# liangxuy/ReGenNet

Hardware: AMD Instinct MI355X
Metric: sampled motions/sec (higher is better)
Workload: dtype bf16 MFMA operands, fp32 accumulate/LayerNorm/softmax, for 990 of 1000 steps; fp16 MFMA operands for the next 8; split-bf16 (x3) for the last 2; 1 GPU; ntu: [B=256/GPU,56,6,60] online/concat/no_cond L8 d512, 1000-step DDPM, Philox noise, hipGraph=on; batch_per_gpu=256, global_batch=256, denoiser_evals_per_motion=1000, parallelism=batch-shard x1

## Files before the change

### regennet_amd/csrc/rgn_device.h

```cpp
#pragma once
#include <hip/hip_runtime.h>

#include <type_traits>
#include <utility>

#include "rgn_internal.h"
#include "rgn_layout.h"

#define RGN_AS1 __attribute__((address_space(1)))
#define RGN_AS3 __attribute__((address_space(3)))

namespace rgn {
namespace {

template <class T, int N>
using vec_t = T __attribute__((ext_vector_type(N)));
typedef vec_t<float, 2> f32x2;
typedef vec_t<float, 4> f32x4;
typedef vec_t<float, 16> f32x16;
typedef vec_t<__bf16, 2> bf16x2;
typedef vec_t<__bf16, 4> bf16x4;
typedef vec_t<__bf16, 8> bf16x8;
typedef vec_t<_Float16, 2> f16x2;
typedef vec_t<_Float16, 8> f16x8;
typedef vec_t<unsigned int, 2> u32x2;
typedef vec_t<unsigned int, 4> u32x4;

template <int N>
__device__ __forceinline__ void wait_vmcnt() {
    asm volatile("s_waitcnt vmcnt(%0)" ::"n"(N > 63 ? 63 : N) : "memory");
}
template <int N>
__device__ __forceinline__ void wait_lgkmcnt() {
    static_assert(N >= 0 && N <= 15, "lgkmcnt is a four-bit counter");
    asm volatile("s_waitcnt lgkmcnt(%0)" ::"n"(N) : "memory");
}

template <int CTRL>
__device__ __forceinline__ float dpp(float v) {
    return __builtin_bit_cast(float, __builtin_amdgcn_update_dpp(0, __builtin_bit_cast(int, v), CTRL, 0xf, 0xf, true));
}
__device__ __forceinline__ float row16_sum(float v) {
    v += dpp<0xB1>(v);
    v += dpp<0x4E>(v);
    v += dpp<0x141>(v);
    v += dpp<0x140>(v);
    return v;
}
__device__ __forceinline__ float wave_sum_dpp(float v) {
    const int b = __builtin_bit_cast(int, row16_sum(v));
    return __builtin_bit_cast(float, __builtin_amdgcn_readlane(b, 0)) + __builtin_bit_cast(float, __builtin_amdgcn_readlane(b, 16)) +
           __builtin_bit_cast(float, __builtin_amdgcn_readlane(b, 32)) + __builtin_bit_cast(float, __builtin_amdgcn_readlane(b, 48));
}
__device__ __forceinline__ float wave_sum_shfl(float v) {
#pragma unroll
    for (int o = 32; o > 0; o >>= 1) v += __shfl_xor(v, o, 64);
    return v;
}
__device__ __forceinline__ float wave_max_shfl(float v) {
#pragma unroll
    for (int o = 32; o > 0; o >>= 1) v = fmaxf(v, __shfl_xor(v, o, 64));
    return v;
}

template <int... Is, class F>
__device__ __forceinline__ void static_for_seq(std::integer_sequence<int, Is...>, F&& f) { (f(std::integral_constant<int, Is>{}), ...); }
template <int N, class F>
__device__ __forceinline__ void static_for(F&& f) { static_for_seq(std::make_integer_sequence<int, N>{}, static_cast<F&&>(f)); }

__device__ __forceinline__ void split_bf16(const f32x4 v, bf16x4& hi, bf16x4& lo) {
#pragma unroll
    for (int j = 0; j < 4; ++j) {
        const __bf16 h = (__bf16)v[j];
        hi[j] = h;
        lo[j] = (__bf16)(v[j] - (float)h);
    }
}
__device__ __forceinline__ void split_bf16(const float (&v)[8], bf16x8& hi, bf16x8& lo) {
#pragma unroll
    for (int j = 0; j < 8; ++j) {
        hi[j] = (__bf16)v[j];
        lo[j] = (__bf16)(v[j] - (float)hi[j]);
    }
}
__device__ __forceinline__ void plane_put(const Planes& p, int row, int col, float v) {
    const size_t o = plane_off(p.rows, row, col);
    const __bf16 h = (__bf16)v;
    p.hi[o] = h;
    if (p.lo) p.lo[o] = (__bf16)(v - (float)h);
}

__device__ __forceinline__ float erf_as(float x) {
    const float ax = fabsf(x);
    const float t = __frcp_rn(fmaf(0.3275911f, ax, 1.0f));
    float p = fmaf(1.061405429f, t, -1.453152027f);
    p = fmaf(p, t, 1.421413741f);
    p = fmaf(p, t, -0.284496736f);
    p = fmaf(p, t, 0.254829592f);
    const float e = 1.0f - p * t * __expf(-ax * ax);
    return copysignf(e, x);
}
__device__ __forceinline__ float erf_as_rcpf(float x) {
    const float ax = fabsf(x);
    const float t = __builtin_amdgcn_rcpf(fmaf(0.3275911f, ax, 1.0f));
    float p = fmaf(1.061405429f, t, -1.453152027f);
    p = fmaf(p, t, 1.421413741f);
    p = fmaf(p, t, -0.284496736f);
    p = fmaf(p, t, 0.254829592f);
    const float e = 1.0f - p * t * __expf(-ax * ax);
    return copysignf(e, x);
}
__device__ __forceinline__ float gelu_as(float v) { return v * 0.5f * (1.0f + erf_as(v * 0.70710678118654752440f)); }
__device__ __forceinline__ float gelu_as_rcpf(float v) { return v * 0.5f * (1.0f + erf_as_rcpf(v * 0.70710678118654752440f)); }

__device__ __forceinline__ f32x2 gelu2_p13(f32x2 x) {
    const f32x2 t = {__builtin_amdgcn_fmed3f(x[0], -3.9f, 3.9f), __builtin_amdgcn_fmed3f(x[1], -3.9f, 3.9f)};
    const f32x2 z = t * t;
    f32x2 p = f32x2{3.214928057e-08f, 3.214928057e-08f};
    p = __builtin_elementwise_fma(p, z, f32x2{-2.075321845e-06f, -2.075321845e-06f});
    p = __builtin_elementwise_fma(p, z, f32x2{5.740237248e-05f, 5.740237248e-05f});
    p = __builtin_elementwise_fma(p, z, f32x2{-9.056383278e-04f, -9.056383278e-04f});
    p = __builtin_elementwise_fma(p, z, f32x2{9.218782187e-03f, 9.218782187e-03f});
    p = __builtin_elementwise_fma(p, z, f32x2{-6.556465477e-02f, -6.556465477e-02f});
    p = __builtin_elementwise_fma(p, z, f32x2{3.986084461e-01f, 3.986084461e-01f});
    return x * __builtin_elementwise_fma(t, p, f32x2{0.5f, 0.5f});
}
__device__ __forceinline__ f32x2 gelu2_p15(f32x2 x) {
    f32x2 u = x * 0.70710678118654752440f;
    u = __builtin_elementwise_min(__builtin_elementwise_max(u, f32x2{-3.2f, -3.2f}), f32x2{3.2f, 3.2f});
    const f32x2 z = u * u;
    f32x2 p = f32x2{-2.6911866e-07f, -2.6911866e-07f};
    p = __builtin_elementwise_fma(p, z, f32x2{1.2661994e-05f, 1.2661994e-05f});
    p = __builtin_elementwise_fma(p, z, f32x2{-2.5566161e-04f, -2.5566161e-04f});
    p = __builtin_elementwise_fma(p, z, f32x2{2.9286479e-03f, 2.9286479e-03f});
    p = __builtin_elementwise_fma(p, z, f32x2{-2.1317327e-02f, -2.1317327e-02f});
    p = __builtin_elementwise_fma(p, z, f32x2{1.0528564e-01f, 1.0528564e-01f});
    p = __builtin_elementwise_fma(p, z, f32x2{-3.7135834e-01f, -3.7135834e-01f});
    p = __builtin_elementwise_fma(p, z, f32x2{1.1274883e+00f, 1.1274883e+00f});
    const f32x2 hx = x * 0.5f;
    return __builtin_elementwise_fma(hx, p * u, hx);
}

template <bool F16> struct OpFmt;
template <> struct OpFmt<false> {
    typedef __bf16 t;
    typedef __bf16 v8 __attribute__((ext_vector_type(8)));
    typedef __bf16 v4 __attribute__((ext_vector_type(4)));
    typedef float acc16 __attribute__((ext_vector_type(16)));
    static __device__ __forceinline__ acc16 mfma(v8 a, v8 b, acc16 c) { return __builtin_amdgcn_mfma_f32_32x32x16_bf16(a, b, c, 0, 0, 0); }
};
template <> struct OpFmt<true> {
    typedef _Float16 t;
    typedef _Float16 v8 __attribute__((ext_vector_type(8)));
    typedef _Float16 v4 __attribute__((ext_vector_type(4)));
    typedef float acc16 __attribute__((ext_vector_type(16)));
    static __device__ __forceinline__ acc16 mfma(v8 a, v8 b, acc16 c) { return __builtin_amdgcn_mfma_f32_32x32x16_f16(a, b, c, 0, 0, 0); }
};

__device__ __forceinline__ int xcd_affine(int bid, int nwg) {
    const int q8 = nwg >> 3, r8 = nwg & 7, xcd = bid & 7;
    return (xcd < r8 ? xcd * (q8 + 1) : r8 * (q8 + 1) + (xcd - r8) * q8) + (bid >> 3);
}

__device__ __forceinline__ void half_swap(float& a, float& b) { asm volatile("s_nop 1\n\tv_permlane32_swap_b32 %0, %1\n\ts_nop 1" : "+v"(a), "+v"(b)); }
__device__ __forceinline__ float half_max(float v) {
    float o = v;
    asm volatile("" : "+v"(o));
    half_swap(v, o);
    return fmaxf(v, o);
}
__device__ __forceinline__ float half_sum(float v) {
    float o = v;
    asm volatile("" : "+v"(o));
    half_swap(v, o);
    return v + o;
}

template <int AUX = 0, int NKB = 16, int NW = 8, class T>
__device__ __forceinline__ void tile_dma_in(char* img, const T* plane, int rows, size_t row0, int live, int lane, int wave) {
    const int r16 = lane >> 2, c = lane & 3;
#pragma unroll
    for (int j = 0; j < 4 * NKB / NW; ++j) {
        const int p = wave + NW * j, kb = p >> 2, r = (p & 3) * 16 + r16;
        const int rr = r < live ? r : live - 1;
        const size_t src = plane_chunk(rows, row0 + rr, kb, img_dma_chunk(r, c));
        __builtin_amdgcn_global_load_lds((const RGN_AS1 void*)(plane + src), (RGN_AS3 void*)(img + p * 1024), 16, 0, AUX);
    }
}

__device__ __forceinline__ void rot6d_to_matrix(float a1x, float a1y, float a1z, float a2x, float a2y, float a2z, float* m) {
    float n1 = fmaxf(sqrtf(a1x * a1x + a1y * a1y + a1z * a1z), 1e-12f);
    const float b1x = a1x / n1, b1y = a1y / n1, b1z = a1z / n1;
    const float dot = b1x * a2x + b1y * a2y + b1z * a2z;
    float b2x = a2x - dot * b1x, b2y = a2y - dot * b1y, b2z = a2z - dot * b1z;
    const float n2 = fmaxf(sqrtf(b2x * b2x + b2y * b2y + b2z * b2z), 1e-12f);
    b2x /= n2; b2y /= n2; b2z /= n2;
    m[0] = b1x; m[1] = b1y; m[2] = b1z;
    m[3] = b2x; m[4] = b2y; m[5] = b2z;
    m[6] = b1y * b2z - b1z * b2y;
    m[7] = b1z * b2x - b1x * b2z;
    m[8] = b1x * b2y - b1y * b2x;
}

template <class F>
auto dispatch_bools(F&& f) { return f(); }
template <class F, class... Rest>
auto dispatch_bools(F&& f, bool b, Rest... rest) {
    auto bind = [&](auto B) { return dispatch_bools([&](auto... bs) { return f(B, bs...); }, rest...); };
    return b ? bind(std::true_type{}) : bind(std::false_type{});
}

}
}
```

### regennet_amd/csrc/rgn_layers.hip

```cpp
#include "rgn_internal.h"
#include "rgn_device.h"
#include "rgn_tail.h"
#include "rgn_sampler.h"

#include <hip/hip_runtime.h>

#include <cmath>
#include <type_traits>
#include <utility>

namespace rgn {

#ifndef RGN_LY_ST_AUX
#define RGN_LY_ST_AUX 16
#endif

constexpr int LY_NTH = 512, LY_KB = 4096;
constexpr int LY_X = 0, LY_Y = 64 * 1024, LY_EXCH = LY_Y, LY_RED = 128 * 1024, LY_REDF = 2 * 8 * 64, LY_VEC = LY_RED + 2 * LY_REDF * 4, LY_VECW = 640,
              LY_LDS = 160 * 1024;
constexpr int LY_PF = LY_VEC + 8 * LY_VECW * 4;
static_assert(LY_PF + 8 * 256 <= LY_LDS, "LDS map");
enum { V_BO = 0, V_G1 = 64, V_G2 = 128, V_B2 = 192, V_SPV = 256, V_BF1 = 320 , V_BF2 = 448, V_G3 = 512, V_B3 = 576 };
constexpr int LY_RDA = 6;
constexpr int LY_RDM = 8;
struct LYT {
    static constexpr int MT = 2, NT = 2, NW = 8, R = 64, RD = LY_RDM, KB = LY_KB, RED = LY_RED, REDF = LY_REDF;
};

#ifdef RGN_LY_STAMPS
__device__ long long g_ly_st[1024][16];
#define RGN_LYT(i)                                                                                   \
    {                                                                                                \
        __builtin_amdgcn_sched_barrier(0);                                                           \
        if (threadIdx.x == 0 && blockIdx.x < 1024 && l == RGN_LY_STAMPS) g_ly_st[blockIdx.x][i] = __builtin_readcyclecounter(); \
        __builtin_amdgcn_sched_barrier(0);                                                           \
    }
#define RGN_LYS(i)                                                                                   \
    {                                                                                                \
        __builtin_amdgcn_sched_barrier(0);                                                           \
        if (threadIdx.x == 0 && blockIdx.x < 1024 && it == 1) g_ly_st[blockIdx.x][i] = __builtin_readcyclecounter(); \
        __builtin_amdgcn_sched_barrier(0);                                                           \
    }
#else
#define RGN_LYT(i)
#define RGN_LYS(i)
#endif

constexpr int LY_XLD = 356, LY_TILE = 0, LY_XIMG = 92160, LY_NKX = 11;
static_assert(64 * LY_XLD * 4 <= LY_XIMG && LY_XIMG + LY_NKX * 4096 <= LY_LDS, "step boundary LDS map");

template <bool STEPS, bool GUIDED = false, bool F16 = false, bool INPAINT = false>
__global__ __launch_bounds__(LY_NTH, 2) void k_layers(LayersArgs g) {
    static_assert(STEPS || !GUIDED, "guidance inside the launch needs the step boundary");
    static_assert(STEPS || !INPAINT, "in-painting (rgn_set_inpainting) belongs to the step boundary");
    using OP = OpFmt<F16>;
    using op_t = typename OP::t;
    using op8 = typename OP::v8;
    using op4 = typename OP::v4;
    extern __shared__ __attribute__((aligned(16))) char smem[];
    const int tid = threadIdx.x, lane = tid & 63;
    const int wave = __builtin_amdgcn_readfirstlane(tid >> 6);
    const int wn = wave & 3, hg = wave >> 2;
    const int l31 = lane & 31, kh = lane >> 5;
    const int b = xcd_affine(blockIdx.x, gridDim.x), Tq = g.Tq;
    const size_t row0 = (size_t)b * Tq;
#ifdef RGN_LY_PRIO
    if (wave >= 4) __builtin_amdgcn_s_setprio(RGN_LY_PRIO);
#endif
    float* vec = reinterpret_cast<float*>(smem + LY_VEC) + wave * LY_VECW;
    const int lane16 = lane * 16;
    tile_dma_in(smem + LY_X, g.h, g.rows, row0, Tq, lane, wave);
    const int first_step = (g.stepvec || STEPS) ? *g.d_step : 0;
    const TailLane tl = tail_lane<LYT>(smem, lane, wave);
    static_assert(LY_X == 0, "a_off addresses the image at byte 0");
    int a_off[2], a_offy[2];
    tail_a_off(a_off, lane);
    tail_a_off(a_offy, a_off, LY_Y);
    using Pass = TailPass;
    op8 wf[LY_RDM][2];
    const float qs2 = g.qscale * 1.44269504088896340736f;

    f32x4 qb[4];
    float vb1;
    auto load_qbias = [&](const float* bqkv, int r) {
        const float* bq = bqkv + (2 * r + hg) * 128 + wn * 32;
#pragma unroll
        for (int i4 = 0; i4 < 4; ++i4) qb[i4] = *reinterpret_cast<const f32x4*>(bq + 8 * i4 + 4 * kh);
        vb1 = bq[1024 + l31];
    };

    wait_vmcnt<0>();
    __builtin_amdgcn_s_barrier();
    load_qbias(g.lw[0].bqkv, 0);

    const int nit = STEPS ? g.steps : 1;
    auto out_proj = [&](f32x16 (&acc)[2][2], int wv) {
#pragma unroll
        for (int a2 = 0; a2 < 2; ++a2)
#pragma unroll
            for (int b2 = 0; b2 < 2; ++b2)
#pragma unroll
                for (int i = 0; i < 16; ++i) acc[a2][b2][i] = 0.f;
        if (wv < 6) {
            const int cb0 = 2 * wv;
            const Pass p_out{__builtin_amdgcn_make_buffer_rsrc(const_cast<__bf16*>(g.Wout) + (size_t)cb0 * 1024, 0, (16 * g.nb_out - cb0) * 2048, 0x00020000), LY_NKX * 2048, 0};
#pragma unroll
            for (int s2 = 0; s2 < LY_RDM - 1; ++s2) tail_load_g<OP, LYT>(wf, tl, p_out, s2, s2);
            tail_gemm<OP, LYT, 32, false, 0>(acc, wf, tl, a_off, p_out, p_out);
        }
    };
    for (int it = 0; it < nit; ++it) {
    const int step = first_step - it;
    for (int pass = 0; pass < (GUIDED ? 2 : 1); ++pass) {
    if (GUIDED && pass == 1) {
        f32x16 accp[2][2];
        int wave_p = wave, lane_p = lane, b_p = b;
        asm volatile("" : "+s"(wave_p), "+s"(b_p));
        asm volatile("" : "+v"(lane_p));
        out_proj(accp, wave_p);
        if (wave_p < 6) {
            float* pk = g.park + ((size_t)b_p * 6 + wave_p) * 4096 + lane_p * 4;
#pragma unroll
            for (int nt = 0; nt < 2; ++nt)
#pragma unroll
                for (int mt = 0; mt < 2; ++mt)
#pragma unroll
                    for (int i4 = 0; i4 < 4; ++i4)
                        *reinterpret_cast<f32x4*>(pk + ((nt * 2 + mt) * 4 + i4) * 256) = f32x4{accp[nt][mt][4 * i4], accp[nt][mt][4 * i4 + 1], accp[nt][mt][4 * i4 + 2], accp[nt][mt][4 * i4 + 3]};
        }
        __builtin_amdgcn_s_barrier();
        tile_dma_in<16>(smem + LY_X, g.h, g.rows, g.half + (size_t)b_p * Tq, Tq, lane_p, wave_p);
        wait_vmcnt<0>();
        __builtin_amdgcn_s_barrier();
    }
    for (int l = 0; l < g.L; ++l) {
        const LayerWts& w = g.lw[l];
        RGN_LYT(0)
        op4 attk[2][2][4];
        float bo_r = 0.f;
        {
            struct PassA { __amdgpu_buffer_rsrc_t rs; };
            auto qrs = [&](int r) {
                const int blk = (2 * r + hg) * 4 + wn;
                return __builtin_amdgcn_make_buffer_rsrc(const_cast<__bf16*>(w.Wqkv) + (size_t)blk * 1024, 0, 3 * 512 * 512 * 2 - blk * 2048, 0x00020000);
            };
            const PassA pa[2] = {{qrs(0)}, {qrs(1)}};
            op8 wq[LY_RDA][3];
            auto load_ga = [&](const PassA& ps, int hs, int slot) {
                int soff;
                asm volatile("s_mov_b32 %0, %1" : "=s"(soff) : "i"(frag_granule(hs, 48 * 2048)));
#pragma unroll
                for (int t = 0; t < 3; ++t)
                    wq[slot][t] = __builtin_bit_cast(op8, __builtin_amdgcn_raw_buffer_load_b128(ps.rs, lane16, soff + t * (16 * 2048), 0));
            };
            constexpr int AH = LY_RDA - 1;
#pragma unroll
            for (int s = 0; s < AH; ++s) load_ga(pa[0], s, s);
#pragma unroll
            for (int r = 0; r < 2; ++r) {
                const int head = 2 * r + hg;
                f32x16 acc[2][3];
#pragma unroll
                for (int ta = 0; ta < 2; ++ta)
#pragma unroll
                    for (int i4 = 0; i4 < 4; ++i4)
#pragma unroll
                        for (int e = 0; e < 4; ++e) {
                            acc[ta][0][4 * i4 + e] = qb[i4][e];
                            acc[ta][1][4 * i4 + e] = 0.f;
                            acc[ta][2][4 * i4 + e] = vb1;
                        }
                __builtin_amdgcn_sched_barrier(0);
                {
                    op8 af[2];
#pragma unroll
                    for (int ta = 0; ta < 2; ++ta) af[ta] = *reinterpret_cast<const op8*>(smem + a_off[0] + ta * 2048);
#pragma unroll
                    for (int hs = 0; hs < 32; ++hs) {
                        op8 afn[2];
#pragma unroll
                        for (int ta = 0; ta < 2; ++ta) {
                            afn[ta] = af[ta];
                            if (hs + 1 < 32) afn[ta] = *reinterpret_cast<const op8*>(smem + ((hs + 1) >> 1) * LY_KB + a_off[(hs + 1) & 1] + ta * 2048);
                        }
                        if (hs + AH < 32) load_ga(pa[r], hs + AH, (32 * r + hs + AH) % LY_RDA);
                        else if (r == 0) load_ga(pa[1], hs + AH - 32, (32 * r + hs + AH) % LY_RDA);
                        if (hs + AH < 32 || r == 0) {
                            if (hs < AH) wait_vmcnt<3 * AH + 5>();
                            else wait_vmcnt<3 * AH>();
                        }
                        const int slot = (32 * r + hs) % LY_RDA;
#pragma unroll
                        for (int t = 0; t < 3; ++t)
#pragma unroll
                            for (int ta = 0; ta < 2; ++ta) {
                                if (t < 2) acc[ta][t] = OP::mfma(wq[slot][t], af[ta], acc[ta][t]);
                                else acc[ta][t] = OP::mfma(af[ta], wq[slot][t], acc[ta][t]);
                            }
#pragma unroll
                        for (int ta = 0; ta < 2; ++ta) af[ta] = afn[ta];
                    }
                }
                __builtin_amdgcn_sched_barrier(0);
                RGN_LYT(1 + 3 * r)
                op8 qh[2][2], kf[2][2], vh[2][2];
#pragma unroll
                for (int ta = 0; ta < 2; ++ta)
#pragma unroll
                    for (int sl = 0; sl < 2; ++sl)
#pragma unroll
                        for (int j = 0; j < 8; ++j) {
                            const int i = 8 * sl + j;
                            qh[ta][sl][j] = (op_t)acc[ta][0][i];
                            kf[ta][sl][j] = (op_t)acc[ta][1][i];
                            vh[ta][sl][j] = (op_t)acc[ta][2][i];
                        }
                if (r == 0) load_qbias(w.bqkv, 1);
                else bo_r = w.bo[64 * wave + lane];
                f32x16 st[3];
#pragma unroll
                for (int tl = 0; tl < 3; ++tl) {
                    const int kj = tl >> 1, qtile = tl ? 1 : 0;
#pragma unroll
                    for (int i = 0; i < 16; ++i) st[tl][i] = 0.f;
#pragma unroll
                    for (int sl = 0; sl < 2; ++sl) st[tl] = OP::mfma(kf[kj][sl], qh[qtile][sl], st[tl]);
                }
                f32x4* sred = reinterpret_cast<f32x4*>(smem + LY_EXCH);
#pragma unroll
                for (int tl = 0; tl < 3; ++tl)
#pragma unroll
                    for (int i4 = 0; i4 < 4; ++i4) {
                        const f32x4 v = {st[tl][4 * i4], st[tl][4 * i4 + 1], st[tl][4 * i4 + 2], st[tl][4 * i4 + 3]};
                        sred[(((hg * 3 + tl) * 4 + wn) * 4 + i4) * 64 + lane] = v;
                    }
                if (r == 0) { RGN_LYT(12) }
                wait_lgkmcnt<0>();
                __builtin_amdgcn_s_barrier();
                if (r == 0) { RGN_LYT(13) }
                {
                    const int kg = lane & 3, qi = lane >> 2, qt = qi >> 3, ql = 8 * wn + (qi & 7), Q = 32 * qt + ql;
                    const int kj = kg >> 1, sl = kg & 1;
                    const bool live = !(qt == 0 && kj == 1);
                    const int tl = live ? qt + kj : 0;
                    const char* ex = smem + LY_EXCH + ((hg * 3 + tl) * 4 * 4 + 2 * sl) * 1024 + ql * 16;
                    f32x4 sv[4];
#pragma unroll
                    for (int a2 = 0; a2 < 2; ++a2)
#pragma unroll
                        for (int h2 = 0; h2 < 2; ++h2) {
                            f32x4 v = *reinterpret_cast<const f32x4*>(ex + a2 * 1024 + h2 * 512);
#pragma unroll
                            for (int ww = 1; ww < 4; ++ww) {
                                const f32x4 u = *reinterpret_cast<const f32x4*>(ex + ww * 4096 + a2 * 1024 + h2 * 512);
#pragma unroll
                                for (int e = 0; e < 4; ++e) v[e] += u[e];
                            }
                            sv[2 * a2 + h2] = v;
                        }
                    int xlim = live ? (Q < Tq - 1 ? Q : Tq - 1) - 32 * kj - 16 * sl : -1;
                    asm volatile("" : "+v"(xlim));
                    float mx = -INFINITY;
#pragma unroll
                    for (int c4 = 0; c4 < 4; ++c4)
#pragma unroll
                        for (int e = 0; e < 4; ++e) {
                            sv[c4][e] = (4 * c4 + e <= xlim) ? sv[c4][e] : -INFINITY;
                            mx = fmaxf(mx, sv[c4][e]);
                        }
                    mx = fmaxf(mx, __builtin_bit_cast(float, __builtin_amdgcn_mov_dpp(__builtin_bit_cast(int, mx), 0xB1, 0xf, 0xf, true)));
                    mx = fmaxf(mx, __builtin_bit_cast(float, __builtin_amdgcn_mov_dpp(__builtin_bit_cast(int, mx), 0x4E, 0xf, 0xf, true)));
                    float sum = 0.f;
                    const float nmx = -mx * qs2;
#pragma unroll
                    for (int c4 = 0; c4 < 4; ++c4)
#pragma unroll
                        for (int e = 0; e < 4; ++e) {
                            sv[c4][e] = __builtin_amdgcn_exp2f(__builtin_fmaf(sv[c4][e], qs2, nmx));
                            sum += sv[c4][e];
                        }
                    sum += __builtin_bit_cast(float, __builtin_amdgcn_mov_dpp(__builtin_bit_cast(int, sum), 0xB1, 0xf, 0xf, true));
                    sum += __builtin_bit_cast(float, __builtin_amdgcn_mov_dpp(__builtin_bit_cast(int, sum), 0x4E, 0xf, 0xf, true));
                    const float inv = 1.0f / sum;
                    if (live) {
#pragma unroll
                        for (int h2 = 0; h2 < 2; ++h2) {
                            op8 pp;
#pragma unroll
                            for (int e = 0; e < 4; ++e) {
                                pp[e] = (op_t)(sv[h2][e] * inv);
                                pp[4 + e] = (op_t)(sv[2 + h2][e] * inv);
                            }
                            *reinterpret_cast<op8*>(smem + LY_EXCH + (((hg * 3 + tl) * 4 + 0) * 4 + sl) * 1024 + (h2 * 32 + ql) * 16) = pp;
                        }
                    }
                }
                if (r == 0) { RGN_LYT(14) }
                wait_lgkmcnt<0>();
                __builtin_amdgcn_s_barrier();
                if (r == 0) { RGN_LYT(15) }
#pragma unroll
                for (int qtile = 0; qtile < 2; ++qtile) {
                    f32x16 oa;
#pragma unroll
                    for (int i = 0; i < 16; ++i) oa[i] = 0.f;
#pragma unroll
                    for (int tl = qtile; tl <= 2 * qtile; ++tl) {
                        const int kj = tl >> 1;
#pragma unroll
                        for (int sl = 0; sl < 2; ++sl) {
                            const op8 ph = *reinterpret_cast<const op8*>(smem + LY_EXCH + (((hg * 3 + tl) * 4 + 0) * 4 + sl) * 1024 + lane * 16);
                            oa = OP::mfma(vh[kj][sl], ph, oa);
                        }
                    }
#pragma unroll
                    for (int i4 = 0; i4 < 4; ++i4)
#pragma unroll
                        for (int e = 0; e < 4; ++e) attk[r][qtile][i4][e] = (op_t)oa[4 * i4 + e];
                }
                RGN_LYT(2 + 3 * r)
                wait_lgkmcnt<0>();
                __builtin_amdgcn_s_barrier();
                RGN_LYT(3 + 3 * r)
            }
        }
        const Pass p_wo{tail_wrs(w.Wo, 2 * wave, 512 * 512 * 2), 16 * 2048, 0}, p_w1a{tail_wrs(w.W1, 2 * wave, 1024 * 512 * 2), 32 * 2048, 0},
            p_w1b{tail_wrs(w.W1, 16 + 2 * wave, 1024 * 512 * 2), 32 * 2048, 0}, p_w2a{tail_wrs(w.W2, 2 * wave, 512 * 1024 * 2), 16 * 2048, 0},
            p_w2b{p_w2a.rs, 16 * 2048, 32};
        vec[V_BO + lane] = bo_r;
#pragma unroll
        for (int s = 0; s < LY_RDM - 1; ++s) tail_load_g<OP, LYT>(wf, tl, p_wo, s, s);
        int cw = 64 * wave + lane;
        asm volatile("" : "+v"(cw));
        float vv[12];
        {
            const float* src[9] = {w.bo, w.g1, w.g2, w.b2, w.bf1, w.bf1 + 512, w.bf2, w.g3, w.b3};
            vv[1] = src[1][cw]; vv[2] = src[2][cw]; vv[3] = src[3][cw];
            vv[4] = w.b1[cw] + (g.stepvec ? g.stepvec[(size_t)step * g.ldstep + (size_t)l * 512 + cw] : 0.f) +
                    (g.pervec ? g.pervec[((size_t)b + (size_t)pass * g.B) * g.ldper + (size_t)l * 512 + cw] : 0.f);
            vv[5] = src[4][cw]; vv[6] = src[5][cw]; vv[7] = src[6][cw]; vv[8] = src[7][cw]; vv[9] = src[8][cw];
        }
        asm volatile("" ::: "memory");
#pragma unroll
        for (int r = 0; r < 2; ++r)
#pragma unroll
            for (int qtile = 0; qtile < 2; ++qtile)
#pragma unroll
                for (int i4 = 0; i4 < 4; ++i4)
                    *reinterpret_cast<op4*>(smem + LY_Y + ((2 * r + hg) * 4 + wn) * LY_KB + (32 * qtile + l31) * 64 + img_slot(i4, tl.swz) + 8 * kh) = attk[r][qtile][i4];
        wait_lgkmcnt<0>();
        __builtin_amdgcn_s_barrier();
        f32x16 acc[2][2];
        tail_init_bias<LYT>(acc, tl, vec + V_BO);
        RGN_LYT(7)
        tail_gemm<OP, LYT, 32, true, 11>(acc, wf, tl, a_offy, p_wo, p_w1a);
        RGN_LYT(8)
        vec[V_G1 + lane] = vv[1]; vec[V_G2 + lane] = vv[2]; vec[V_B2 + lane] = vv[3]; vec[V_SPV + lane] = vv[4];
        vec[V_BF1 + lane] = vv[5]; vec[V_BF1 + 64 + lane] = vv[6]; vec[V_BF2 + lane] = vv[7]; vec[V_G3 + lane] = vv[8]; vec[V_B3 + lane] = vv[9];
        tail_add_resid<OP, LYT>(acc, tl, LY_X);
        tail_layernorm<LYT, 0>(acc, tl, vec + V_G1, tail_rowvec(tl, vec + V_SPV));
        tail_layernorm<LYT, 1>(acc, tl, vec + V_G2, tail_rowvec(tl, vec + V_B2));
        tail_store_img<OP, LYT>(acc, tl, LY_X);
        wait_lgkmcnt<0>();
        __builtin_amdgcn_s_barrier();
        RGN_LYT(9)
        f32x16 acc2[2][2];
        tail_ffn<OP, LYT>(acc2, wf, tl, a_off, a_offy, LY_Y, p_w1a, p_w1b, p_w2a, p_w2b, vec + V_BF1, vec + V_BF2);
        load_qbias(g.lw[l + 1 < g.L ? l + 1 : 0].bqkv, 0);
#ifndef RGN_LY_NO_PREFETCH
        if constexpr (STEPS) {
            if (l == g.L - 1) {
                const int nsl = (int)(gridDim.x >> 3) >= 32 ? 32 : ((int)(gridDim.x >> 3) > 0 ? (int)(gridDim.x >> 3) : 1);
                const int sl = (int)(blockIdx.x >> 3) % nsl;
                const int n_out = 16 * g.nb_out * 16, n_all = n_out + LY_NKX * 16 * 16;
                const unsigned pf_lds = (unsigned)(size_t)((RGN_AS3 char*)(smem + LY_PF)) + (unsigned)wave * 256u;
                for (int ln = sl + nsl * tid; ln < n_all; ln += nsl * LY_NTH) {
                    const char* pp = ln < n_out ? reinterpret_cast<const char*>(g.Wout) + (size_t)ln * 128 : reinterpret_cast<const char*>(g.Wx) + (size_t)(ln - n_out) * 128;
                    int m0_keep;
                    asm volatile("s_mov_b32 %0, m0\n\ts_mov_b32 m0, %2\n\ts_nop 0\n\tglobal_load_lds_dword %1, off\n\ts_mov_b32 m0, %0" : "=&s"(m0_keep) : "v"(pp), "s"(pf_lds) : "memory");
                }
            }
        }
#endif
        RGN_LYT(10)
        tail_add_resid<OP, LYT>(acc2, tl, LY_X);
        tail_layernorm<LYT, 0>(acc2, tl, vec + V_G3, tail_rowvec(tl, vec + V_B3));
        tail_store_img<OP, LYT>(acc2, tl, LY_X);
        wait_lgkmcnt<0>();
        __builtin_amdgcn_s_barrier();
        RGN_LYT(11)
    }
    }
    if constexpr (STEPS) {
        int lane_s = lane, wave_s = wave, b_s = b;
        asm volatile("" : "+v"(lane_s));
        asm volatile("" : "+s"(wave_s), "+s"(b_s));
        const int l31_s = lane_s & 31, kh_s = lane_s >> 5;
        const size_t row0_s = (size_t)b_s * Tq;
        auto col4s = [&](int nt, int i4) { return 32 * nt + 8 * i4 + 4 * kh_s; };
        RGN_LYS(12)
        const SampleParams sp = *g.sp;
        const StepCoef k = g.tab[step];
        const int T = Tq, gb = g.s0 + b_s;
        const float gscale = GUIDED ? g.scale[gb] : 0.f;
        const __amdgpu_buffer_rsrc_t park_rs = __builtin_amdgcn_make_buffer_rsrc(GUIDED ? g.park + ((size_t)b_s * 6 + (wave_s < 6 ? wave_s : 0)) * 4096 : nullptr, 0, 4096 * 4, 0x00020000);
        f32x16 acc[2][2];
        out_proj(acc, wave_s);
        __builtin_amdgcn_s_barrier();
        float* tile = reinterpret_cast<float*>(smem + LY_TILE);
#pragma unroll
        for (int nt = 0; nt < 2; ++nt)
#pragma unroll
            for (int i4 = 0; i4 < 4; ++i4) {
                const int n = 64 * wave_s + col4s(nt, i4);
                if (n < 352) {
                    f32x4 bb = {0.f, 0.f, 0.f, 0.f};
                    if (n < g.F) bb = *reinterpret_cast<const f32x4*>(g.bout + n);
#pragma unroll
                    for (int mt = 0; mt < 2; ++mt) {
                        f32x4 v = {acc[nt][mt][4 * i4] + bb[0], acc[nt][mt][4 * i4 + 1] + bb[1], acc[nt][mt][4 * i4 + 2] + bb[2], acc[nt][mt][4 * i4 + 3] + bb[3]};
                        if constexpr (GUIDED) {
                            const f32x4 cc = __builtin_bit_cast(f32x4, __builtin_amdgcn_raw_buffer_load_b128(park_rs, (lane_s * 4 + ((nt * 2 + mt) * 4 + i4) * 256) * 4, 0, 16));
#pragma unroll
                            for (int e = 0; e < 4; ++e) v[e] = guide(cc[e] + bb[e], v[e], gscale);
                        }
                        *reinterpret_cast<f32x4*>(tile + (32 * mt + l31_s) * LY_XLD + n) = v;
                    }
                }
            }
        const Pass p_wx{__builtin_amdgcn_make_buffer_rsrc(const_cast<__bf16*>(g.Wx) + (size_t)(2 * wave_s) * 1024, 0, (LY_NKX * 16 - 2 * wave_s) * 2048, 0x00020000), 16 * 2048, 0};
#pragma unroll
        for (int s2 = 0; s2 < LY_RDM - 1; ++s2) tail_load_g<OP, LYT>(wf, tl, p_wx, s2, s2);
        op4 c0v[2][2][4];
#pragma unroll
        for (int mt = 0; mt < 2; ++mt) {
            const int r = 32 * mt + l31_s, rr = r < T ? r : T - 1;
#pragma unroll
            for (int nt = 0; nt < 2; ++nt)
#pragma unroll
                for (int i4 = 0; i4 < 4; ++i4)
                    c0v[nt][mt][i4] = *reinterpret_cast<const op4*>(g.c0 + (row0_s + rr) * 512 + 64 * wave_s + col4s(nt, i4));
        }
        op4 c0u[GUIDED ? 2 : 1][2][4];
        if constexpr (GUIDED) {
#pragma unroll
            for (int mt = 0; mt < 2; ++mt) {
                const int r = 32 * mt + l31_s, rr = r < T ? r : T - 1;
#pragma unroll
                for (int nt = 0; nt < 2; ++nt)
#pragma unroll
                    for (int i4 = 0; i4 < 4; ++i4)
                        c0u[nt][mt][i4] = *reinterpret_cast<const op4*>(g.c0 + ((size_t)g.half + row0_s + rr) * 512 + 64 * wave_s + col4s(nt, i4));
            }
        }
        wait_lgkmcnt<0>();
        __builtin_amdgcn_s_barrier();
        RGN_LYS(13)
        {
            const int t = lane_s;
            const bool valid = t < T;
            const size_t FT = (size_t)g.F * T;
            const int bn = noise_motion(sp, gb);
            char* ximg = smem + LY_XIMG;
            const int q = lane_s & 3, tq = t - q;
            const bool run4 = valid && (tq & 3) == 0 && tq + 3 < T;
            const bool quads = !sp.noise && !g.no_quads && __all(run4 || tq >= T);
            float xpre[LY_NKX][4];
#pragma unroll
            for (int i2 = 0; i2 < LY_NKX; ++i2)
#pragma unroll
                for (int j = 0; j < 4; ++j) {
                    const int f = 4 * (wave_s + 8 * i2) + j;
                    xpre[i2][j] = (valid && f < g.F) ? sp.x[(size_t)gb * FT + (size_t)f * T + t] : 0.f;
                }
            const int ximg_lane = img_run(lane_s, wave_s >> 1, wave_s & 1);
            constexpr int LY_IPD = GUIDED ? 1 : 2;
            unsigned char mpre[INPAINT ? LY_NKX : 1][4];
            float ipre[INPAINT ? LY_NKX : 1][4];
            const InpaintRsrc irs = inpaint_rsrc(sp, INPAINT ? (size_t)gb * FT : 0, INPAINT ? FT : 0);
            auto inp_request = [&](auto IG) __attribute__((always_inline)) {
                constexpr int ig = decltype(IG)::value;
                if constexpr (INPAINT && ig < LY_NKX) {
#pragma unroll
                    for (int j = 0; j < 4; ++j) inpaint_load(irs, t, (4 * (wave_s + 8 * ig) + j) * T, mpre[ig][j], ipre[ig][j]);
                    asm volatile("" ::: "memory");
                }
            };
            static_for<LY_IPD>([&](auto IG) __attribute__((always_inline)) { inp_request(IG); });
            auto update4 = [&](int i2, int fg, const float (&eps_in)[4], const float (&xv)[4]) {
                op4 nvb;
#pragma unroll
                for (int j = 0; j < 4; ++j) nvb[j] = (op_t)0.f;
                if (valid && 4 * fg < g.F) {
                    const f32x4 x04 = *reinterpret_cast<const f32x4*>(tile + lane_s * LY_XLD + 4 * fg);
#pragma unroll
                    for (int j = 0; j < 4; ++j) {
                        const int f = 4 * fg + j;
                        unsigned char im = 0;
                        float iv = 0.f;
                        if constexpr (INPAINT) { im = mpre[i2][j]; iv = ipre[i2][j]; }
                        const float x0 = pred_x0<INPAINT>(x04[j], im, iv, sp.clip);
                        const size_t o = (size_t)gb * FT + (size_t)f * T + t;
// ... 122 lines not shown
```

### regennet_amd/csrc/rgn_layout.h

```cpp
#pragma once
#include <cstddef>
#include <cstdint>
#include <cstring>

#if defined(__HIP__) || defined(__CUDACC__)
#define RGN_HD __attribute__((host)) __attribute__((device))
#else
#define RGN_HD
#endif

namespace rgn {

template <class T> struct layout_index { typedef T type; };

template <class I = size_t>
RGN_HD constexpr inline I plane_chunk(typename layout_index<I>::type rows, typename layout_index<I>::type row, int kb, int chunk) {
    return ((I)kb * rows + row) * 32 + chunk * 8;
}
template <class I = size_t>
RGN_HD constexpr inline I plane_off(typename layout_index<I>::type rows, typename layout_index<I>::type row, int col) {
    return ((I)(col >> 5) * rows + row) * 32 + (col & 31);
}

RGN_HD constexpr inline int img_swz(int row) { return (row >> 2) & 3; }
RGN_HD constexpr inline int img_slot(int chunk, int swz) { return (chunk ^ swz) << 4; }
RGN_HD constexpr inline int img_chunk(int row, int chunk) { return row * 64 + img_slot(chunk, img_swz(row)); }
RGN_HD constexpr inline int img_frag(int row, int ks, int kh) { return row * 64 + img_slot(2 * ks + kh, img_swz(row)); }
RGN_HD constexpr inline int img_run(int row, int i4, int kh) { return row * 64 + img_slot(i4, img_swz(row)) + 8 * kh; }
RGN_HD constexpr inline int img_dma_chunk(int row, int slot) { return slot ^ img_swz(row); }

RGN_HD constexpr inline int frag_lane(int n, int k) { return 32 * ((k % 16) / 8) + n % 32; }
RGN_HD constexpr inline int frag_elem(int k) { return k % 8; }
RGN_HD constexpr inline size_t frag_off(size_t nb_all, int n, int k) {
    return ((((size_t)(k / 32) * nb_all + n / 32) * 2 + (k % 32) / 16) * 64 + frag_lane(n, k)) * 8 + frag_elem(k);
}
RGN_HD constexpr inline int frag_granule(int hs, int kstride) { return (hs >> 1) * kstride + (hs & 1) * 1024; }

RGN_HD constexpr inline int mfma32_row(int i, int kh) { return (i & 3) + 8 * (i >> 2) + 4 * kh; }
RGN_HD constexpr inline int mfma32_col(int lane) { return lane & 31; }

RGN_HD constexpr inline size_t attn_slab_base(int H, int Tqp, int dh, size_t b, int hd) { return (b * H + hd) * Tqp * dh; }
RGN_HD constexpr inline size_t attn_slab_off(int H, int Tqp, int dh, size_t b, int hd, int t, int c) { return ((b * H + hd) * Tqp + t) * dh + c; }

inline uint16_t f2bf(float f) {
    uint32_t u;
    memcpy(&u, &f, 4);
    if ((u & 0x7fffffffu) > 0x7f800000u) return (uint16_t)((u >> 16) | 0x40);
    u += 0x7fffu + ((u >> 16) & 1u);
    return (uint16_t)(u >> 16);
}
inline float bf2f(uint16_t h) {
    uint32_t u = (uint32_t)h << 16;
    float f;
    memcpy(&f, &u, 4);
    return f;
}

namespace layout_detail {
constexpr bool chunks_permute() {
    for (int r = 0; r < 64; ++r) {
        int seen = 0;
        for (int c = 0; c < 4; ++c) {
            seen |= 1 << ((img_chunk(r, c) - r * 64) >> 4);
            if (img_chunk(r, img_dma_chunk(r, c)) != r * 64 + c * 16) return false;
        }
        if (seen != 15) return false;
    }
    return true;
}
constexpr bool roles_agree() {
    for (int r = 0; r < 64; ++r)
        for (int ks = 0; ks < 2; ++ks)
            for (int kh = 0; kh < 2; ++kh) {
                if (img_frag(r, ks, kh) != img_chunk(r, 2 * ks + kh)) return false;
                if (img_run(r, 2 * ks + kh, 1) != img_chunk(r, 2 * ks + kh) + 8) return false;
            }
    return true;
}
constexpr bool cd_rows_permute() {
    unsigned seen = 0;
    for (int i = 0; i < 16; ++i)
        for (int kh = 0; kh < 2; ++kh) seen |= 1u << mfma32_row(i, kh);
    return seen == 0xffffffffu;
}
}
static_assert(layout_detail::chunks_permute(), "the chunk map permutes 0 .. 3 in every row and the DMA source rule inverts it");
static_assert(layout_detail::roles_agree(), "fragment (r, ks, kh) is logical chunk 2 ks + kh; an accumulator run is half a chunk");
static_assert(layout_detail::cd_rows_permute(), "the C/D row map covers the 32 rows of a tile");
static_assert(plane_off(300, 7, 37) == plane_chunk(300, 7, 1, 0) + 5, "a plane element lies in chunk (col % 32) / 8 of k-block col / 32");
static_assert(attn_slab_off(4, 64, 128, 3, 2, 0, 0) == attn_slab_base(4, 64, 128, 3, 2) && attn_slab_base(4, 64, 128, 3, 2) == (size_t)(3 * 4 + 2) * 64 * 128, "a head's slab is Tqp x dh elements, heads of a sample back to back");
static_assert(attn_slab_off(4, 64, 128, 3, 2, 59, 127) + 1 == attn_slab_off(4, 64, 128, 3, 2, 60, 0), "a token row of a head is dh contiguous elements");
static_assert(frag_off(16, 33, 49) * 2 == frag_granule(3, 16 * 2048) + 2048 + frag_lane(33, 49) * 16 + frag_elem(49) * 2, "granule, column block, lane, element");

}
```

Before: 486.8 motions/s.

## Restructure attention to per-wave 16x16 MFMA tiles over swizzled LDS Q/K/V images

Each wave now writes its Q, K and V^T accumulator fragments into bank-conflict-free swizzled LDS images. Each wave then computes full-key scores, the causal softmax and P·V for its own 16-query block using 16x16x32 MFMAs. This removes the cross-wave partial-score reduction through LDS and two of the three barriers per head round. Causal work is balanced by a reversed query-block assignment for the second head group. The cost is extra LDS image traffic and reshaped output stores, plus new cross-lane reductions via permlane16/32 swaps.

```diff
diff --git a/regennet_amd/csrc/rgn_device.h b/regennet_amd/csrc/rgn_device.h
--- a/regennet_amd/csrc/rgn_device.h
+++ b/regennet_amd/csrc/rgn_device.h
@@ -148,6 +148,7 @@
     typedef __bf16 v4 __attribute__((ext_vector_type(4)));
     typedef float acc16 __attribute__((ext_vector_type(16)));
     static __device__ __forceinline__ acc16 mfma(v8 a, v8 b, acc16 c) { return __builtin_amdgcn_mfma_f32_32x32x16_bf16(a, b, c, 0, 0, 0); }
+    static __device__ __forceinline__ f32x4 mfma16(v8 a, v8 b, f32x4 c) { return __builtin_amdgcn_mfma_f32_16x16x32_bf16(a, b, c, 0, 0, 0); }
 };
 template <> struct OpFmt<true> {
     typedef _Float16 t;
@@ -155,6 +156,7 @@
     typedef _Float16 v4 __attribute__((ext_vector_type(4)));
     typedef float acc16 __attribute__((ext_vector_type(16)));
     static __device__ __forceinline__ acc16 mfma(v8 a, v8 b, acc16 c) { return __builtin_amdgcn_mfma_f32_32x32x16_f16(a, b, c, 0, 0, 0); }
+    static __device__ __forceinline__ f32x4 mfma16(v8 a, v8 b, f32x4 c) { return __builtin_amdgcn_mfma_f32_16x16x32_f16(a, b, c, 0, 0, 0); }
 };
 
 __device__ __forceinline__ int xcd_affine(int bid, int nwg) {
@@ -174,6 +176,20 @@
     asm volatile("" : "+v"(o));
     half_swap(v, o);
     return v + o;
+}
+
+__device__ __forceinline__ void row_pair_swap(float& a, float& b) { asm volatile("s_nop 1\n\tv_permlane16_swap_b32 %0, %1\n\ts_nop 1" : "+v"(a), "+v"(b)); }
+__device__ __forceinline__ float quarter_max(float v) {
+    float o = v;
+    asm volatile("" : "+v"(o));
+    row_pair_swap(v, o);
+    return half_max(fmaxf(v, o));
+}
+__device__ __forceinline__ float quarter_sum(float v) {
+    float o = v;
+    asm volatile("" : "+v"(o));
+    row_pair_swap(v, o);
+    return half_sum(v + o);
 }
 
 template <int AUX = 0, int NKB = 16, int NW = 8, class T>
diff --git a/regennet_amd/csrc/rgn_layers.hip b/regennet_amd/csrc/rgn_layers.hip
--- a/regennet_amd/csrc/rgn_layers.hip
+++ b/regennet_amd/csrc/rgn_layers.hip
@@ -16,8 +16,9 @@
 #endif
 
 constexpr int LY_NTH = 512, LY_KB = 4096;
-constexpr int LY_X = 0, LY_Y = 64 * 1024, LY_EXCH = LY_Y, LY_RED = 128 * 1024, LY_REDF = 2 * 8 * 64, LY_VEC = LY_RED + 2 * LY_REDF * 4, LY_VECW = 640,
+constexpr int LY_X = 0, LY_Y = 64 * 1024, LY_ATT = LY_Y, LY_AIMG = 16 * 1024, LY_RED = 128 * 1024, LY_REDF = 2 * 8 * 64, LY_VEC = LY_RED + 2 * LY_REDF * 4, LY_VECW = 640,
               LY_LDS = 160 * 1024;
+static_assert(LY_ATT + 2 * 3 * LY_AIMG == LY_LDS, "the attention images (two heads x q | k | v^T) fill Y and the 32 KiB behind it");
 constexpr int LY_PF = LY_VEC + 8 * LY_VECW * 4;
 static_assert(LY_PF + 8 * 256 <= LY_LDS, "LDS map");
 enum { V_BO = 0, V_G1 = 64, V_G2 = 128, V_B2 = 192, V_SPV = 256, V_BF1 = 320 , V_BF2 = 448, V_G3 = 512, V_B3 = 576 };
@@ -136,7 +137,7 @@
     for (int l = 0; l < g.L; ++l) {
         const LayerWts& w = g.lw[l];
         RGN_LYT(0)
-        op4 attk[2][2][4];
+        op4 attk[2][8];
         float bo_r = 0.f;
         {
             struct PassA { __amdgpu_buffer_rsrc_t rs; };
@@ -203,127 +204,105 @@
                 }
                 __builtin_amdgcn_sched_barrier(0);
                 RGN_LYT(1 + 3 * r)
-                op8 qh[2][2], kf[2][2], vh[2][2];
+                int lane_a = lane;
+                asm volatile("" : "+v"(lane_a));
+                const int l31_a = lane_a & 31, kh_a = lane_a >> 5, lq = lane_a & 15, g4 = lane_a >> 4;
+                char* const imq = smem + LY_ATT + hg * (3 * LY_AIMG);
+                if (r == 1) {
+                    wait_lgkmcnt<0>();
+                    __builtin_amdgcn_s_barrier();
+                }
 #pragma unroll
                 for (int ta = 0; ta < 2; ++ta)
 #pragma unroll
-                    for (int sl = 0; sl < 2; ++sl)
+                    for (int s = 0; s < 2; ++s) {
+                        op8 qv, kv, vv;
 #pragma unroll
                         for (int j = 0; j < 8; ++j) {
-                            const int i = 8 * sl + j;
-                            qh[ta][sl][j] = (op_t)acc[ta][0][i];
-                            kf[ta][sl][j] = (op_t)acc[ta][1][i];
-                            vh[ta][sl][j] = (op_t)acc[ta][2][i];
-                        }
+                            qv[j] = (op_t)acc[ta][0][8 * s + j];
+                            kv[j] = (op_t)acc[ta][1][8 * s + j];
+                        }
+#pragma unroll
+                        for (int e = 0; e < 4; ++e) {
+                            vv[e] = (op_t)acc[ta][2][4 * s + e];
+                            vv[4 + e] = (op_t)acc[ta][2][8 + 4 * s + e];
+                        }
+                        const int qk_off = att_qk_chunk(32 * ta + l31_a, wn, 2 * kh_a + s);
+                        *reinterpret_cast<op8*>(imq + qk_off) = qv;
+                        *reinterpret_cast<op8*>(imq + LY_AIMG + qk_off) = kv;
+                        *reinterpret_cast<op8*>(imq + 2 * LY_AIMG + att_vt_chunk(32 * wn + l31_a, ta, 2 * s + kh_a)) = vv;
+                    }
                 if (r == 0) load_qbias(w.bqkv, 1);
                 else bo_r = w.bo[64 * wave + lane];
-                f32x16 st[3];
-#pragma unroll
-                for (int tl = 0; tl < 3; ++tl) {
-                    const int kj = tl >> 1, qtile = tl ? 1 : 0;
-#pragma unroll
-                    for (int i = 0; i < 16; ++i) st[tl][i] = 0.f;
-#pragma unroll
-                    for (int sl = 0; sl < 2; ++sl) st[tl] = OP::mfma(kf[kj][sl], qh[qtile][sl], st[tl]);
-                }
-                f32x4* sred = reinterpret_cast<f32x4*>(smem + LY_EXCH);
-#pragma unroll
-                for (int tl = 0; tl < 3; ++tl)
-#pragma unroll
-                    for (int i4 = 0; i4 < 4; ++i4) {
-                        const f32x4 v = {st[tl][4 * i4], st[tl][4 * i4 + 1], st[tl][4 * i4 + 2], st[tl][4 * i4 + 3]};
-                        sred[(((hg * 3 + tl) * 4 + wn) * 4 + i4) * 64 + lane] = v;
-                    }
-                if (r == 0) { RGN_LYT(12) }
+                if (!STEPS && r == 0) { RGN_LYT(12) }
                 wait_lgkmcnt<0>();
                 __builtin_amdgcn_s_barrier();
-                if (r == 0) { RGN_LYT(13) }
-                {
-                    const int kg = lane & 3, qi = lane >> 2, qt = qi >> 3, ql = 8 * wn + (qi & 7), Q = 32 * qt + ql;
-                    const int kj = kg >> 1, sl = kg & 1;
-                    const bool live = !(qt == 0 && kj == 1);
-                    const int tl = live ? qt + kj : 0;
-                    const char* ex = smem + LY_EXCH + ((hg * 3 + tl) * 4 * 4 + 2 * sl) * 1024 + ql * 16;
-                    f32x4 sv[4];
-#pragma unroll
-                    for (int a2 = 0; a2 < 2; ++a2)
-#pragma unroll
-                        for (int h2 = 0; h2 < 2; ++h2) {
-                            f32x4 v = *reinterpret_cast<const f32x4*>(ex + a2 * 1024 + h2 * 512);
-#pragma unroll
-                            for (int ww = 1; ww < 4; ++ww) {
-                                const f32x4 u = *reinterpret_cast<const f32x4*>(ex + ww * 4096 + a2 * 1024 + h2 * 512);
-#pragma unroll
-                                for (int e = 0; e < 4; ++e) v[e] += u[e];
-                            }
-                            sv[2 * a2 + h2] = v;
-                        }
-                    int xlim = live ? (Q < Tq - 1 ? Q : Tq - 1) - 32 * kj - 16 * sl : -1;
+                if (!STEPS && r == 0) { RGN_LYT(13) }
+                const int jq = hg ? 3 - wn : wn;
+                auto attend = [&](auto NPC) __attribute__((always_inline)) {
+                    constexpr int NP = decltype(NPC)::value;
+                    op8 qf[4];
+#pragma unroll
+                    for (int c = 0; c < 4; ++c) qf[c] = *reinterpret_cast<const op8*>(imq + jq * 4096 + att_qk_chunk(lq, c, g4));
+                    f32x4 st[2 * NP];
+#pragma unroll
+                    for (int kb = 0; kb < 2 * NP; ++kb) st[kb] = f32x4{0.f, 0.f, 0.f, 0.f};
+#pragma unroll
+                    for (int c = 0; c < 4; ++c)
+#pragma unroll
+                        for (int kb = 0; kb < 2 * NP; ++kb) {
+                            const op8 kf = *reinterpret_cast<const op8*>(imq + LY_AIMG + kb * 4096 + att_qk_chunk(lq, c, g4));
+                            st[kb] = OP::mfma16(kf, qf[c], st[kb]);
+                        }
+                    const int Q = 16 * jq + lq;
+                    int xlim = (Q < Tq - 1 ? Q : Tq - 1) - 4 * g4;
                     asm volatile("" : "+v"(xlim));
                     float mx = -INFINITY;
 #pragma unroll
-                    for (int c4 = 0; c4 < 4; ++c4)
-#pragma unroll
-                        for (int e = 0; e < 4; ++e) {
-                            sv[c4][e] = (4 * c4 + e <= xlim) ? sv[c4][e] : -INFINITY;
-                            mx = fmaxf(mx, sv[c4][e]);
-                        }
-                    mx = fmaxf(mx, __builtin_bit_cast(float, __builtin_amdgcn_mov_dpp(__builtin_bit_cast(int, mx), 0xB1, 0xf, 0xf, true)));
-                    mx = fmaxf(mx, __builtin_bit_cast(float, __builtin_amdgcn_mov_dpp(__builtin_bit_cast(int, mx), 0x4E, 0xf, 0xf, true)));
+                    for (int kb = 0; kb < 2 * NP; ++kb)
+#pragma unroll
+                        for (int i = 0; i < 4; ++i) {
+                            st[kb][i] = (16 * kb + i <= xlim) ? st[kb][i] : -INFINITY;
+                            mx = fmaxf(mx, st[kb][i]);
+                        }
+                    mx = quarter_max(mx);
                     float sum = 0.f;
                     const float nmx = -mx * qs2;
 #pragma unroll
-                    for (int c4 = 0; c4 < 4; ++c4)
-#pragma unroll
-                        for (int e = 0; e < 4; ++e) {
-                            sv[c4][e] = __builtin_amdgcn_exp2f(__builtin_fmaf(sv[c4][e], qs2, nmx));
-                            sum += sv[c4][e];
-                        }
-                    sum += __builtin_bit_cast(float, __builtin_amdgcn_mov_dpp(__builtin_bit_cast(int, sum), 0xB1, 0xf, 0xf, true));
-                    sum += __builtin_bit_cast(float, __builtin_amdgcn_mov_dpp(__builtin_bit_cast(int, sum), 0x4E, 0xf, 0xf, true));
-                    const float inv = 1.0f / sum;
-                    if (live) {
-#pragma unroll
-                        for (int h2 = 0; h2 < 2; ++h2) {
-                            op8 pp;
-#pragma unroll
-                            for (int e = 0; e < 4; ++e) {
-                                pp[e] = (op_t)(sv[h2][e] * inv);
-                                pp[4 + e] = (op_t)(sv[2 + h2][e] * inv);
-                            }
-                            *reinterpret_cast<op8*>(smem + LY_EXCH + (((hg * 3 + tl) * 4 + 0) * 4 + sl) * 1024 + (h2 * 32 + ql) * 16) = pp;
-                        }
+                    for (int kb = 0; kb < 2 * NP; ++kb)
+#pragma unroll
+                        for (int i = 0; i < 4; ++i) {
+                            st[kb][i] = __builtin_amdgcn_exp2f(__builtin_fmaf(st[kb][i], qs2, nmx));
+                            sum += st[kb][i];
+                        }
+                    const float inv = 1.0f / quarter_sum(sum);
+                    f32x4 oa[8];
+#pragma unroll
+                    for (int d = 0; d < 8; ++d) oa[d] = f32x4{0.f, 0.f, 0.f, 0.f};
+#pragma unroll
+                    for (int p = 0; p < NP; ++p) {
+                        op8 pp;
+#pragma unroll
+                        for (int i = 0; i < 4; ++i) {
+                            pp[i] = (op_t)(st[2 * p][i] * inv);
+                            pp[4 + i] = (op_t)(st[2 * p + 1][i] * inv);
+                        }
+#pragma unroll
+                        for (int d = 0; d < 8; ++d) oa[d] = OP::mfma16(*reinterpret_cast<const op8*>(imq + 2 * LY_AIMG + d * 2048 + att_vt_chunk(lq, p, g4)), pp, oa[d]);
                     }
-                }
-                if (r == 0) { RGN_LYT(14) }
-                wait_lgkmcnt<0>();
-                __builtin_amdgcn_s_barrier();
-                if (r == 0) { RGN_LYT(15) }
-#pragma unroll
-                for (int qtile = 0; qtile < 2; ++qtile) {
-                    f32x16 oa;
-#pragma unroll
-                    for (int i = 0; i < 16; ++i) oa[i] = 0.f;
-#pragma unroll
-                    for (int tl = qtile; tl <= 2 * qtile; ++tl) {
-                        const int kj = tl >> 1;
-#pragma unroll
-                        for (int sl = 0; sl < 2; ++sl) {
-                            const op8 ph = *reinterpret_cast<const op8*>(smem + LY_EXCH + (((hg * 3 + tl) * 4 + 0) * 4 + sl) * 1024 + lane * 16);
-                            oa = OP::mfma(vh[kj][sl], ph, oa);
-                        }
-                    }
-#pragma unroll
-                    for (int i4 = 0; i4 < 4; ++i4)
-#pragma unroll
-                        for (int e = 0; e < 4; ++e) attk[r][qtile][i4][e] = (op_t)oa[4 * i4 + e];
-                }
+#pragma unroll
+                    for (int d = 0; d < 8; ++d)
+#pragma unroll
+                        for (int e = 0; e < 4; ++e) attk[r][d][e] = (op_t)oa[d][e];
+                };
+                if (jq >= 2) attend(std::integral_constant<int, 2>{});
+                else attend(std::integral_constant<int, 1>{});
                 RGN_LYT(2 + 3 * r)
-                wait_lgkmcnt<0>();
-                __builtin_amdgcn_s_barrier();
-                RGN_LYT(3 + 3 * r)
             }
         }
+        wait_lgkmcnt<0>();
+        __builtin_amdgcn_s_barrier();
+        RGN_LYT(6)
         const Pass p_wo{tail_wrs(w.Wo, 2 * wave, 512 * 512 * 2), 16 * 2048, 0}, p_w1a{tail_wrs(w.W1, 2 * wave, 1024 * 512 * 2), 32 * 2048, 0},
             p_w1b{tail_wrs(w.W1, 16 + 2 * wave, 1024 * 512 * 2), 32 * 2048, 0}, p_w2a{tail_wrs(w.W2, 2 * wave, 512 * 1024 * 2), 16 * 2048, 0},
             p_w2b{p_w2a.rs, 16 * 2048, 32};
@@ -341,13 +320,16 @@
             vv[5] = src[4][cw]; vv[6] = src[5][cw]; vv[7] = src[6][cw]; vv[8] = src[7][cw]; vv[9] = src[8][cw];
         }
         asm volatile("" ::: "memory");
-#pragma unroll
-        for (int r = 0; r < 2; ++r)
-#pragma unroll
-            for (int qtile = 0; qtile < 2; ++qtile)
-#pragma unroll
-                for (int i4 = 0; i4 < 4; ++i4)
-                    *reinterpret_cast<op4*>(smem + LY_Y + ((2 * r + hg) * 4 + wn) * LY_KB + (32 * qtile + l31) * 64 + img_slot(i4, tl.swz) + 8 * kh) = attk[r][qtile][i4];
+        {
+            int lane_y = lane;
+            asm volatile("" : "+v"(lane_y));
+            const int gy = lane_y >> 4, row = 16 * (hg ? 3 - wn : wn) + (lane_y & 15);
+#pragma unroll
+            for (int r = 0; r < 2; ++r)
+#pragma unroll
+                for (int d = 0; d < 8; ++d)
+                    *reinterpret_cast<op4*>(smem + LY_Y + ((2 * r + hg) * 4 + (d >> 1)) * LY_KB + img_run(row, 2 * (d & 1) + (gy >> 1), gy & 1)) = attk[r][d];
+        }
         wait_lgkmcnt<0>();
         __builtin_amdgcn_s_barrier();
         f32x16 acc[2][2];
diff --git a/regennet_amd/csrc/rgn_layout.h b/regennet_amd/csrc/rgn_layout.h
--- a/regennet_amd/csrc/rgn_layout.h
+++ b/regennet_amd/csrc/rgn_layout.h
@@ -42,6 +42,10 @@
 RGN_HD constexpr inline size_t attn_slab_base(int H, int Tqp, int dh, size_t b, int hd) { return (b * H + hd) * Tqp * dh; }
 RGN_HD constexpr inline size_t attn_slab_off(int H, int Tqp, int dh, size_t b, int hd, int t, int c) { return ((b * H + hd) * Tqp + t) * dh + c; }
 
+RGN_HD constexpr inline int att_qk_chunk(int t, int c, int g) { return t * 256 + (((4 * c + g) ^ (t & 15)) << 4); }
+RGN_HD constexpr inline int att_vt_swz(int dh) { return ((dh >> 1) & 7) ^ ((dh & 1) << 2); }
+RGN_HD constexpr inline int att_vt_chunk(int dh, int p, int g) { return dh * 128 + (((4 * p + g) ^ att_vt_swz(dh)) << 4); }
+
 inline uint16_t f2bf(float f) {
     uint32_t u;
     memcpy(&u, &f, 4);
@@ -83,10 +87,36 @@
         for (int kh = 0; kh < 2; ++kh) seen |= 1u << mfma32_row(i, kh);
     return seen == 0xffffffffu;
 }
+constexpr bool att_images_conflict_free() {
+    const int first[4] = {0, 4, 32, 36};
+    for (int grp = 0; grp < 4; ++grp)
+        for (int x = 0; x < 4; ++x) {
+            unsigned qk = 0, vt = 0;
+            for (int n = 0; n < 16; ++n) {
+                const int rel = (grp & 1) ? (n < 8 ? n : n < 12 ? n + 4 : n + 12) : (n < 4 ? n : n < 8 ? n + 8 : n + 12);
+                const int lane = first[grp] + rel, row = lane & 15, g = lane >> 4;
+                qk |= 1u << ((att_qk_chunk(row, x, g) >> 4) & 15);
+                vt |= 1u << ((att_vt_chunk(row, x & 1, g) >> 4) & 15);
+            }
+            if (qk != 0xffffu || vt != 0xffffu) return false;
+        }
+    for (int t0 = 0; t0 < 64; t0 += 8)
+        for (int q = 0; q < 16; ++q) {
+            unsigned qk = 0, vt = 0;
+            for (int n = 0; n < 8; ++n) {
+                qk |= 1u << ((att_qk_chunk(t0 + n, q >> 2, q & 3) >> 4) & 7);
+                vt |= 1u << ((att_vt_chunk(t0 + n, (q >> 2) & 1, q & 3) >> 4) & 7);
+            }
+            if (qk != 0xffu || vt != 0xffu) return false;
+        }
+    return true;
+}
 }
 static_assert(layout_detail::chunks_permute(), "the chunk map permutes 0 .. 3 in every row and the DMA source rule inverts it");
 static_assert(layout_detail::roles_agree(), "fragment (r, ks, kh) is logical chunk 2 ks + kh; an accumulator run is half a chunk");
 static_assert(layout_detail::cd_rows_permute(), "the C/D row map covers the 32 rows of a tile");
+static_assert(layout_detail::att_images_conflict_free(), "the attention images: every fragment read and every image store is free of bank conflicts");
+static_assert(att_qk_chunk(16 * 3 + 5, 2, 1) == 3 * 4096 + att_qk_chunk(5, 2, 1) && att_vt_chunk(16 * 7 + 5, 1, 2) == 7 * 2048 + att_vt_chunk(5, 1, 2), "a 16-row block further is a constant further");
 static_assert(plane_off(300, 7, 37) == plane_chunk(300, 7, 1, 0) + 5, "a plane element lies in chunk (col % 32) / 8 of k-block col / 32");
 static_assert(attn_slab_off(4, 64, 128, 3, 2, 0, 0) == attn_slab_base(4, 64, 128, 3, 2) && attn_slab_base(4, 64, 128, 3, 2) == (size_t)(3 * 4 + 2) * 64 * 128, "a head's slab is Tqp x dh elements, heads of a sample back to back");
 static_assert(attn_slab_off(4, 64, 128, 3, 2, 59, 127) + 1 == attn_slab_off(4, 64, 128, 3, 2, 60, 0), "a token row of a head is dh contiguous elements");
```

Result: no change. 488.4 motions/s (median of 6 runs) (+0.3%).
